# ZINZINBIN/Disruption-Prediciton-based-on-Multimodal-Deep-Learning

Hardware: AMD Instinct MI355X
Metric: clips/sec (fwd+bwd) R2Plus1D T=21 128x128 (higher is better)
Workload: dtype f32 storage; products as 3 fp16 (forward) / bf16 (backward) MFMAs on hi+lo splits, f32 accumulate; 1 GPU; R2Plus1D layer_sizes=[1,2,2,1] alpha=0.01, per-GPU clips (8,3,21,128,128) fp32, forward+FocalLoss(gamma=2)+backward+clip_grad_norm(1.0)+AdamW(2e-4), BN in train mode; per_gpu_batch=8, global_batch=8, parallelism=dp1

## Files before the change

disruption-prediciton-based-on-multimodal-deep-learning_amd/csrc/conv_patch.hip:

```cpp
#include "common.h"
#include <cstdlib>

#include "patch_common.h"

template <bool F16, int NT = 256>
__device__ __forceinline__ void stage_image(__amdgpu_buffer_rsrc_t src, int Cpitch, int c0, int cvalid4,
                                            const int* sG, int npix, int C8, unsigned magic, char* img, int pitch,
                                            int lo_off, bool prologue, const float* sScale, const float* sShift,
                                            float pslope, int t, bool presplit = false) {
  const int total = npix * C8;
  for (int base = 0; base < total; base += NT * 4) {
    float4 va[4], vb[4];
    int pix[4], c8s[4];
#pragma unroll
    for (int u = 0; u < 4; ++u) {
      const int item = min(base + u * NT + t, total - 1);
      const int pixel = mdiv(item, magic);
      const int c8 = item - pixel * C8;
      const int gp = sG[pixel];
      const bool in = gp >= 0 && c8 * 2 < cvalid4;
      const unsigned off = in ? (presplit ? (unsigned)(gp * C8 + c8) * 32u : (unsigned)(gp * Cpitch + c0 + c8 * 8) * 4u) : MD_OOB;
      va[u] = buf_load4(src, off);
      vb[u] = buf_load4(src, (in && (presplit || c8 * 2 + 1 < cvalid4)) ? off + 16u : MD_OOB);
      pix[u] = base + u * NT + t < total ? (pixel | (in ? 0 : 0x20000000)) : -1;
// ... 245 lines not shown
    if (fuse) {
      const int c = n0 + (j0 + j) * 16 + li;
      const bool cok = c < g.Cpd;
      const float csc = cok ? bw.scale[c] : 0.f, csh = cok ? bw.shift[c] : 0.f, cmu = cok ? bw.mean[c] : 0.f, cis = cok ? bw.invstd[c] : 0.f;
      float yv[2][4];
#pragma unroll
      for (int a = 0; a < 2; ++a)
#pragma unroll
        for (int r = 0; r < 4; ++r)
          yv[a][r] = __builtin_bit_cast(float, __builtin_amdgcn_raw_buffer_load_b32(yrs, colok ? goff[a][r] : MD_OOB, j * 64, 0));
#pragma unroll
      for (int a = 0; a < 2; ++a)
#pragma unroll
        for (int r = 0; r < 4; ++r) {
          const float pre = fmaf(yv[a][r], csc, csh);
          const float v = (acc[a][j][r] + prev[a][r]) * md_dleaky(pre, bw.slope);
          const float vm = v * gw[a][r];
          s1 += vm; s2 = fmaf(vm, (yv[a][r] - cmu) * cis, s2);
          __builtin_amdgcn_raw_buffer_store_b32(__builtin_bit_cast(unsigned, v), drs, colok ? goff[a][r] : MD_OOB, j * 64, 0);
        }
    } else {
#pragma unroll
      for (int a = 0; a < 2; ++a)
#pragma unroll
        for (int r = 0; r < 4; ++r) {
          const float v = acc[a][j][r];
          const float vm = v * gw[a][r];
          s1 += vm; s2 = fmaf(vm, v, s2);
          __builtin_amdgcn_raw_buffer_store_b32(__builtin_bit_cast(unsigned, v + prev[a][r]), drs, colok ? goff[a][r] : MD_OOB, j * 64, 0);
        }
    }
    if (stat_partial != nullptr) {
      s1 += __shfl_xor(s1, 16); s2 += __shfl_xor(s2, 16);
      s1 += __shfl_xor(s1, 32); s2 += __shfl_xor(s2, 32);
      if (lg == 0 && !dup) {
        red[(wr * 2 + 0) * (PNREP * 16) + (j0 + j) * 16 + li] = s1;
        red[(wr * 2 + 1) * (PNREP * 16) + (j0 + j) * 16 + li] = s2;
      }
    }
  }
  if (stat_partial != nullptr) {
    __syncthreads();
    if (t < ncols && n0 + t < g.Cpd) {
      float s1 = 0.f, s2 = 0.f;
#pragma unroll
      for (int w = 0; w < RG; ++w) {
        s1 += red[(w * 2 + 0) * (PNREP * 16) + t];
        s2 += red[(w * 2 + 1) * (PNREP * 16) + t];
      }
      float* sp = stat_partial + (size_t)blockIdx.x * 2 * g.Cpd;
      sp[n0 + t] = s1;
      sp[g.Cpd + n0 + t] = s2;
    }
  }
}

__device__ __forceinline__ float pack2_weight(const float* __restrict__ w, int n, int tap, int ch, int Cout, int Cin, int kwp,
                                              int kw_real, int shift, int taps_real) {
  const int sx = tap % kwp, row = tap / kwp;
  const int j = ch >> 2, c = ch & 3;
  const int dx = 2 * sx + j + shift;
  if (n < Cout && c < Cin && dx >= 0 && dx < kw_real) return w[((size_t)n * Cin + c) * taps_real + row * kw_real + dx];
  return 0.f;
}


struct ClassSpec { int c[3], tap0[3], kc[3], e[3]; };

static bool patch_build(const MdConvDesc* d, int dgrad, PGeom* out, size_t* lds_bytes, const ClassSpec* cls = nullptr,
                        int pers_wgs = 0, int pm_rows = PM, int npb_force = 0) {
  PGeom g;
  const bool sdg = !cls && dgrad && (d->st != 1 || d->sh != 1 || d->sw != 1);
  g.strided = sdg ? 1 : 0;
  if (sdg && (ilog2_exact(d->st) < 0 || ilog2_exact(d->sh) < 0 || ilog2_exact(d->sw) < 0)) return false;
  g.st = dgrad ? 1 : d->st; g.sh = dgrad ? 1 : d->sh; g.sw = dgrad ? 1 : d->sw;
  g.dst_ = d->st; g.dsh_ = d->sh; g.dsw_ = d->sw;
  g.lt = sdg ? ilog2_exact(d->st) : 0; g.lh = sdg ? ilog2_exact(d->sh) : 0; g.lw = sdg ? ilog2_exact(d->sw) : 0;
  g.oddmask = (g.lt ? ((1 << g.lt) - 1) : 0) | ((g.lh ? ((1 << g.lh) - 1) : 0) << 8) | ((g.lw ? ((1 << g.lw) - 1) : 0) << 16);
  g.kt = d->kt; g.padt = d->pt; g.padh = d->ph; g.padw = d->pw;
  const int cs = dgrad ? d->Cout : d->Cin, cd = dgrad ? d->Cin : d->Cout;
  g.Ts = dgrad ? d->To : d->Ti; g.Hs = dgrad ? d->Ho : d->Hi; g.Ws = dgrad ? d->Wo : d->Wi; g.Cps = md_cpad(cs);
  g.Td = dgrad ? d->Ti : d->To; g.Hd = dgrad ? d->Hi : d->Ho; g.Wd = dgrad ? d->Wi : d->Wo; g.Cpd = md_cpad(cd);
  g.kh = d->kh; g.kw = d->kw; g.khw = d->kh * d->kw; g.taps = d->kt * g.khw;
  if (!dgrad) { g.org_t = -d->pt; g.org_h = -d->ph; g.org_w = -d->pw; }
  else { g.org_t = d->pt - (d->kt - 1); g.org_h = d->ph - (d->kh - 1); g.org_w = d->pw - (d->kw - 1); }
  g.Tdf = g.Td; g.Hdf = g.Hd; g.Wdf = g.Wd; g.dmt = g.dmh = g.dmw = 1; g.dpt = g.dph = g.dpw = 0;
  int kt_eff = d->kt, kh_eff = d->kh;
  if (cls) {
    const int sd[3] = {d->st, d->sh, d->sw};
    int cd_[3];
    const int full[3] = {g.Td, g.Hd, g.Wd};
    for (int i = 0; i < 3; ++i) cd_[i] = full[i] > cls->c[i] ? (full[i] - cls->c[i] + sd[i] - 1) / sd[i] : 0;
    if (cd_[0] < 1 || cd_[1] < 1 || cd_[2] < 1) return false;
    g.Td = cd_[0]; g.Hd = cd_[1]; g.Wd = cd_[2];
    g.dmt = sd[0]; g.dmh = sd[1]; g.dmw = sd[2]; g.dpt = cls->c[0]; g.dph = cls->c[1]; g.dpw = cls->c[2];
    g.kt = cls->kc[0]; g.kh = cls->kc[1]; g.kw = cls->kc[2]; g.khw = g.kh * g.kw; g.taps = g.kt * g.khw;
    g.org_t = cls->e[0] - (cls->kc[0] - 1); g.org_h = cls->e[1] - (cls->kc[1] - 1); g.org_w = cls->e[2] - (cls->kc[2] - 1);
    kt_eff = g.kt; kh_eff = g.kh;
  }
  g.pack2 = 0; g.pk_shift = 0; g.pk_kw = d->kw;
  static const int no_pack2 = getenv("MD_PACK2") && atoi(getenv("MD_PACK2")) == 0;
  int kw_eff = cls ? g.kw : d->kw, sw_eff = g.sw;
  if (!dgrad && !no_pack2 && g.Cps == 4 && d->sw == 2 && (d->Wi & 1) == 0 && d->kw >= 2) {
    const int lo = -((d->pw + 1) / 2);
    const int num = d->kw - 1 - d->pw;
    const int hi = num >= 0 ? num / 2 : -((-num + 1) / 2);
// ... 318 lines not shown
int patch_pack(const MdConvDesc* d, int dgrad, const PatchPlan* p, const float* w, float* out, hipStream_t s) {
  (void)p;
  unsigned char handled = 0;
  const int rc = patch_pack_batch(1, &d, &dgrad, &w, &out, &handled, s);
  return rc ? rc : (handled ? MD_OK : MD_ERR_UNSUPPORTED);
}

static bool pers_can_fuse(const PersVariant& pv);
static PersBwd no_bwd() { PersBwd n; n.yraw = nullptr; n.scale = n.shift = n.mean = n.invstd = nullptr; n.slope = 1.f; return n; }
static int patch_launch_half(const PatchPlan* p, const float* src, const float* ps, const float* psh, float slope, const float* wp,
                             float* dst, float* stat, int accumulate, hipStream_t s, const PersBwd* bw) {
  const PGeom& g = p->gh;
  const PersBwd bwv = bw ? *bw : no_bwd();
  if ((accumulate >> 16) & 1) { if (!p->dgrad || g.pack2) return MD_ERR_UNSUPPORTED; }
  const int boxes = p->N * g.nbt * g.nby * g.nbx;
  int npb = p->half_npb;
  {
    static const int fill = getenv("MD_PATCH_FILL") ? atoi(getenv("MD_PATCH_FILL")) : 128;
    while (npb > 32 && boxes * md_cdiv(g.N16, npb) < 2 * fill) npb = md_round_up(md_cdiv(npb, 2), 16) < 32 ? 32 : md_round_up(md_cdiv(npb, 2), 16);
  }
  dim3 grid(boxes, md_cdiv(g.N16, npb));
  static const int dbg = getenv("MD_DBG") ? atoi(getenv("MD_DBG")) : 0;
  accumulate = (accumulate & 0x10001) | ((dbg & 0xff) << 8);
  const int nrep = npb / 16;
  const size_t lds = p->ldsh;
#define LAUNCH_HALF(F16_, NR_)                                                                                          \
  do {                                                                                                                  \
    static bool set_ = false;                                                                                           \
    if (!set_) {                                                                                                        \
      if (hipFuncSetAttribute((const void*)k_conv_patch<F16_, false, NR_, false, true>,                                 \
                              hipFuncAttributeMaxDynamicSharedMemorySize, 160 * 1024) != hipSuccess)                    \
        return MD_ERR_LAUNCH;                                                                                           \
      set_ = true;                                                                                                      \
    }                                                                                                                   \
    MD_KLAUNCH((k_conv_patch<F16_, false, NR_, false, true>), grid, dim3(256), lds, s, g, src, ps, psh, slope,          \
               (const uint4*)wp, dst, stat, accumulate, npb, bwv);                                                      \
  } while (0)
#define LAUNCH_HALF_NR(F16_)                                                                                            \
  switch (nrep) {                                                                                                       \
    case 2: LAUNCH_HALF(F16_, 2); break;                                                                                \
    case 3: LAUNCH_HALF(F16_, 3); break;                                                                                \
    case 4: LAUNCH_HALF(F16_, 4); break;                                                                                \
    case 5: LAUNCH_HALF(F16_, 5); break;                                                                                \
    case 6: LAUNCH_HALF(F16_, 6); break;                                                                                \
    case 7: LAUNCH_HALF(F16_, 7); break;                                                                                \
    case 8: LAUNCH_HALF(F16_, 8); break;                                                                                \
    default: LAUNCH_HALF(F16_, 9); break;                                                                               \
  }
  if (!p->dgrad) { LAUNCH_HALF_NR(true); } else { LAUNCH_HALF_NR(false); }
  MD_CHECK_LAUNCH();
  return MD_OK;
}

static int patch_launch_one(const PatchPlan* p, const PGeom& g, size_t lds, const PersVariant& pv, const float* src, const float* ps,
                            const float* psh, float slope, const float* wp, float* dst, float* stat, int accumulate,
                            const PersBwd* bw, hipStream_t s) {
  if ((accumulate >> 16) & 1) { if (!p->dgrad || g.pack2) return MD_ERR_UNSUPPORTED; }
  if (pv.on && (!bw || pers_can_fuse(pv))) {
    PersBwd none; none.yraw = nullptr; none.scale = none.shift = none.mean = none.invstd = nullptr; none.slope = 1.f;
    return pers_launch(pv.pg, pv.lds, pv.grid, !p->dgrad, src, ps, psh, slope, wp, dst, stat, accumulate, bw ? *bw : none, s);
  }
  if (pv.on && bw && pv.nsl > 0) {
    for (int k = 0; k < pv.nsl; ++k) {
      const int rc = pers_launch(pv.sl[k], pv.sl_lds[k], pv.grid, false, src, ps, psh, slope, wp, dst, stat, accumulate, *bw, s);
      if (rc != MD_OK) return rc;
    }
    return MD_OK;
  }
  if (bw && !p->dgrad) return MD_ERR_UNSUPPORTED;
  if (p->half && &g == &p->g) return patch_launch_half(p, src, ps, psh, slope, wp, dst, stat, accumulate, s, bw);
  const PersBwd bwv = bw ? *bw : no_bwd();
  int nchunks = md_cdiv(g.N16, PNREP * 16);
  const int boxes = p->N * g.nbt * g.nby * g.nbx;
  {
    static const int fill = getenv("MD_PATCH_FILL") ? atoi(getenv("MD_PATCH_FILL")) : 128;
    int wantc = md_cdiv(fill, boxes);
    if (wantc > g.N16 / 16) wantc = g.N16 / 16;
    if (wantc > nchunks) nchunks = wantc;
  }
  const int npb = md_round_up(md_cdiv(g.N16, nchunks), 16);
  dim3 grid(boxes, md_cdiv(g.N16, npb));
  {
    static const int padkb = getenv("MD_LDS_PAD_KB") ? atoi(getenv("MD_LDS_PAD_KB")) : 0;
    if (padkb && lds + (size_t)padkb * 1024 <= 160 * 1024) lds += (size_t)padkb * 1024; else if (padkb) lds = 160 * 1024;
  }
  static const int dbg = getenv("MD_DBG") ? atoi(getenv("MD_DBG")) : 0;
  accumulate = (accumulate & 0x10001) | ((dbg & 0xff) << 8);
  const int nrep = npb / 16;
  static const int w8_env = getenv("MD_PATCH_W8") ? atoi(getenv("MD_PATCH_W8")) : 1;
  const bool w8 = w8_env && !g.strided && nrep >= 2 && (lds > 80 * 1024 || w8_env == 2);
#define LAUNCH_PATCH(F16_, STR_, NR_, W8_)                                                                              \
  do {                                                                                                                  \
    static bool set_ = false;                                                                                           \
    if (!set_) {                                                                                                        \
      if (hipFuncSetAttribute((const void*)k_conv_patch<F16_, STR_, NR_, W8_>,                                          \
                              hipFuncAttributeMaxDynamicSharedMemorySize, 160 * 1024) != hipSuccess)                    \
        return MD_ERR_LAUNCH;                                                                                           \
      set_ = true;                                                                                                      \
    }                                                                                                                   \
    MD_KLAUNCH((k_conv_patch<F16_, STR_, NR_, W8_>), grid, dim3(W8_ ? 512 : 256), lds, s, g, src, ps, psh, slope,       \
               (const uint4*)wp, dst, stat, accumulate, npb, bwv);                                                      \
  } while (0)
#define LAUNCH_PATCH_NR(F16_, STR_, W8_)                                                                                \
  switch (nrep) {                                                                                                       \
    case 1: LAUNCH_PATCH(F16_, STR_, 1, false); break;                                                                  \
    case 2: LAUNCH_PATCH(F16_, STR_, 2, W8_); break;                                                                    \
    case 3: LAUNCH_PATCH(F16_, STR_, 3, W8_); break;                                                                    \
    case 4: LAUNCH_PATCH(F16_, STR_, 4, W8_); break;                                                                    \
    case 5: LAUNCH_PATCH(F16_, STR_, 5, W8_); break;                                                                    \
    case 6: LAUNCH_PATCH(F16_, STR_, 6, W8_); break;                                                                    \
    case 7: LAUNCH_PATCH(F16_, STR_, 7, W8_); break;                                                                    \
    case 8: LAUNCH_PATCH(F16_, STR_, 8, W8_); break;                                                                    \
    default: LAUNCH_PATCH(F16_, STR_, 9, W8_); break;                                                                   \
  }
  if (!p->dgrad) { if (w8) { LAUNCH_PATCH_NR(true, false, true); } else { LAUNCH_PATCH_NR(true, false, false); } }
  else if (!g.strided) { if (w8) { LAUNCH_PATCH_NR(false, false, true); } else { LAUNCH_PATCH_NR(false, false, false); } }
  else { LAUNCH_PATCH_NR(false, true, false); }
  MD_CHECK_LAUNCH();
  return MD_OK;
}

static bool pers_can_fuse(const PersVariant& pv) {
  static const int maxn = getenv("MD_FUSE_MAXN16") ? atoi(getenv("MD_FUSE_MAXN16")) : 48;
  return pv.on && pv.pg.g.N16 <= maxn && !(pv.pg.g.N16 == 48 && pv.pg.nit > 4) && !(pv.pg.g.N16 > 48 && pv.pg.nit > 4);
}
static bool fuse_per_box(const PersVariant& pv) {
  static const int patch_off = getenv("MD_FUSE_PATCH") && atoi(getenv("MD_FUSE_PATCH")) == 0;
  static const int pers_fallback_on = getenv("MD_FUSE_PERS_FALLBACK") && atoi(getenv("MD_FUSE_PERS_FALLBACK")) == 1;
  if (patch_off) return false;
  if (!pv.on) return true;
  return !pers_can_fuse(pv) && pers_fallback_on;
}
bool patch_can_fuse(const PatchPlan* p) {
  if (!p->dgrad) return false;
  auto ok = [](const PersVariant& pv) { return pers_can_fuse(pv) || (pv.on && pv.nsl > 0) || fuse_per_box(pv); };
  if (!p->ncls) return ok(p->pers);
  for (int c = 0; c < p->ncls; ++c) if (!ok(p->cls[c].pers)) return false;
  return true;
}
int patch_fused_blocks(const PatchPlan* p) {
  auto nb = [&](const PGeom& g, const PersVariant& pv) {
    if (pers_can_fuse(pv) || (pv.on && pv.nsl > 0)) return pers_blocks(pv.pg, pv.grid);
    if (p->half && &g == &p->g) return p->N * p->gh.nbt * p->gh.nby * p->gh.nbx;
// ... 150 lines not shown
```

disruption-prediciton-based-on-multimodal-deep-learning_amd/csrc/conv_pers.hip:

```cpp
#include "patch_common.h"
#include <cstdlib>
#include <cstdio>
#include <type_traits>

__device__ __forceinline__ void buf_store4(__amdgpu_buffer_rsrc_t r, unsigned off, f32x4 v) {
  __builtin_amdgcn_raw_buffer_store_b128(__builtin_bit_cast(__attribute__((__vector_size__(4 * sizeof(unsigned)))) unsigned, v), r, off, 0, 0);
}
__device__ __forceinline__ f32x4 buf_load4v(__amdgpu_buffer_rsrc_t r, unsigned off) {
  return __builtin_bit_cast(f32x4, __builtin_amdgcn_raw_buffer_load_b128(r, off, 0, 0));
}
__device__ __forceinline__ f32x4 buf_load4_pinned(__amdgpu_buffer_rsrc_t r, unsigned off) {
  return __builtin_bit_cast(f32x4, __builtin_amdgcn_raw_buffer_load_b128(r, off, 0, 0));
}

template <bool F16, bool FUSE, int NREP, int MAXI>
__global__ __launch_bounds__(512) void k_conv_pers(
    PersGeom pg, const float* __restrict__ src, const float* __restrict__ pscale, const float* __restrict__ pshift,
    float pslope, const uint4* __restrict__ wp, float* __restrict__ dst, float* __restrict__ stat_partial,
    int accumulate, PersBwd bw) {
  extern __shared__ __attribute__((aligned(16))) char sm[];
  const PGeom& g = pg.g;
  constexpr int NT = 512, TT = 256;
  const int t = threadIdx.x;
  const int wave = __builtin_amdgcn_readfirstlane(t >> 6);
// ... 299 lines not shown
    }
  }
#else
  {
    int* ctr = (int*)(sm + pg.off_sync) + team * 16;
    int target = 0;
    auto team_sync = [&]() {
      target += 4;
      __builtin_amdgcn_fence(__ATOMIC_RELEASE, "workgroup");
      if (lane == 0) __hip_atomic_fetch_add(ctr, 1, __ATOMIC_RELAXED, __HIP_MEMORY_SCOPE_WORKGROUP);
      while (__hip_atomic_load(ctr, __ATOMIC_RELAXED, __HIP_MEMORY_SCOPE_WORKGROUP) < target) __builtin_amdgcn_s_sleep(2);
      __builtin_amdgcn_fence(__ATOMIC_ACQUIRE, "workgroup");
    };
    while (cur < pg.nboxes) {
      do_matrix();
      team_sync();
      do_move();
      team_sync();
      cur += stride;
    }
    __syncthreads();
  }
#endif

  if (stats) {
    float* red = (float*)(sm + pg.off_red);
#pragma unroll
    for (int j = 0; j < NREP; ++j)
#pragma unroll
      for (int r = 0; r < 4; ++r) {
        float a1 = s1[j][r], a2 = s2[j][r];
#pragma unroll
        for (int m = 1; m < 16; m <<= 1) { a1 += __shfl_xor(a1, m); a2 += __shfl_xor(a2, m); }
        if (li == 0) {
          red[(wave * 2 + 0) * (PNREP * 16) + c0 + j * 16 + r] = a1;
          red[(wave * 2 + 1) * (PNREP * 16) + c0 + j * 16 + r] = a2;
        }
      }
    __syncthreads();
    if (t < g.N16 && pg.n0 + t < g.Cpd) {
      float a1 = 0.f, a2 = 0.f;
#pragma unroll
      for (int w = 0; w < 8; ++w) {
        a1 += red[(w * 2 + 0) * (PNREP * 16) + t];
        a2 += red[(w * 2 + 1) * (PNREP * 16) + t];
      }
      float* sp = stat_partial + (size_t)blockIdx.x * 2 * g.Cpd + pg.n0;
      sp[t] = a1;
      sp[g.Cpd + t] = a2;
    }
  }
}

static int pers_num_cus() {
  static int n = 0;
  if (!n) {
    int dev = 0; hipDeviceProp_t p;
    if (hipGetDevice(&dev) == hipSuccess && hipGetDeviceProperties(&p, dev) == hipSuccess && p.multiProcessorCount > 0) n = p.multiProcessorCount;
    else { (void)hipGetLastError(); n = 256; }
  }
  return n;
}

bool pers_finish(PersGeom* pg, size_t* lds_bytes, int* grid) {
  PGeom& g = pg->g;
  pg->nsteps = md_cdiv(g.Kc8, 4);
  { int u = pg->nsteps * 4; while ((u & 3) != 2) ++u; pg->bpitch = u * 16; }
  pg->nboxes = 0;
  pg->n0 = 0; pg->N16w = g.N16;
  pg->patch_bytes = (g.P * g.ppitch + 15) & ~15;
  size_t off = (size_t)2 * pg->patch_bytes;
  pg->off_red = 0;
  if (off < (size_t)8 * 2 * PNREP * 16 * 4) off = (size_t)8 * 2 * PNREP * 16 * 4;
  pg->off_bres = (int)off; off += (size_t)2 * g.N16 * pg->bpitch;
  pg->off_k = (int)off; off += (size_t)(pg->nsteps * 4 + 4) * 4;
  off = (off + 15) & ~(size_t)15;
  pg->off_row = (int)off; off += (size_t)PM * 8;
  pg->sc_stride = g.C8 * 8; pg->bn_stride = g.N16;
  pg->off_sc = (int)off; off += (size_t)2 * pg->sc_stride * 4;
  pg->off_bn = (int)off; off += (size_t)4 * pg->bn_stride * 4;
  off = (off + 15) & ~(size_t)15;
  pg->off_sync = (int)off; off += 128;
  if (off > (size_t)(160 * 1024)) return false;
  *lds_bytes = off;
  *grid = pers_num_cus();
  return true;
}

size_t pers_bres_bytes(int Kc8, int N16) {
  int u = md_cdiv(Kc8, 4) * 4; while ((u & 3) != 2) ++u;
  return (size_t)2 * N16 * u * 16;
}
size_t pers_fixed_bytes(int Cps, int N16) { return (size_t)PM * 8 + (size_t)(2 * (Cps + 8) + 4 * N16) * 4 + 256 + 144; }

int pers_launch(const PersGeom& pg, size_t lds, int grid, bool f16, const float* src, const float* ps, const float* psh, float slope,
                const float* wp, float* dst, float* stat, int accumulate, const PersBwd& bw, hipStream_t s) {
  const PGeom& g = pg.g;
  const int nrep = g.N16 / 16;
  const int nblk = pers_blocks(pg, grid);
  static const int dbg = getenv("MD_DBG") ? atoi(getenv("MD_DBG")) : 0;
  static const int xcd = getenv("MD_PERS_XCD") ? atoi(getenv("MD_PERS_XCD")) : 0;
  static const int early = getenv("MD_PERS_EARLY") ? atoi(getenv("MD_PERS_EARLY")) : 0;
  accumulate = (accumulate & 0x10001) | ((dbg & 0xff) << 8) | (xcd ? 0x40000 : 0) | (early ? 0x80000 : 0);
#define LAUNCH_PERS(F16_, FUSE_, NR_, MX_)                                                                              \
  do {                                                                                                                  \
    static bool set_ = false;                                                                                           \
    if (!set_) {                                                                                                        \
// ... 31 lines not shown
```

disruption-prediciton-based-on-multimodal-deep-learning_amd/csrc/patch_common.h:

```cpp
#pragma once
#include "common.h"

typedef __bf16 bf16x8 __attribute__((ext_vector_type(8)));
typedef __bf16 bf16x2 __attribute__((ext_vector_type(2)));
typedef float f32x2 __attribute__((ext_vector_type(2)));

#define PM 128
#define PNREP 9
#define PB_PITCH 160
#define PMAXC 320

struct PGeom {
  int Ts, Hs, Ws, Cps;
  int Td, Hd, Wd, Cpd;
  int kh, kw, khw, taps;
  int org_t, org_h, org_w;
  int st, sh, sw;
  int strided;
  int dst_, dsh_, dsw_;
  int lt, lh, lw, oddmask;
  int kt, padt, padh, padw;
  int zero_off;
  int bt, by, bx, byx;
  int nbt, nby, nbx;
// ... 62 lines not shown
  } else {
#pragma unroll
    for (int i = 0; i < 4; ++i) {
      const f32x2 x = {v[2 * i], v[2 * i + 1]};
      const f32x2 pre = __builtin_elementwise_fma(x, s[i], h[i]);
      const f32x2 t = pre * sl;
      v[2 * i] = pre[0] > 0.f ? pre[0] : t[0]; v[2 * i + 1] = pre[1] > 0.f ? pre[1] : t[1];
    }
  }
}
__device__ __forceinline__ void zero8(float* v) {
#pragma unroll
  for (int e = 0; e < 8; ++e) v[e] = 0.f;
}

__device__ __forceinline__ int mdiv(int x, unsigned magic) { return magic ? (int)__umulhi((unsigned)x, magic) : x; }

#define MD_OOB 0x80000000u
__device__ __forceinline__ __amdgpu_buffer_rsrc_t make_rsrc(const void* p, unsigned bytes) {
  return __builtin_amdgcn_make_buffer_rsrc(const_cast<void*>(p), 0, bytes, 0x00020000);
}
__device__ __forceinline__ float4 buf_load4(__amdgpu_buffer_rsrc_t r, unsigned off) {
  const f32x4 f = __builtin_bit_cast(f32x4, __builtin_amdgcn_raw_buffer_load_b128(r, off, 0, 0));
  return make_float4(f[0], f[1], f[2], f[3]);
}

template <bool F16>
__device__ __forceinline__ f32x4 mma(uint4 a, uint4 b, f32x4 c) {
  if (F16) return __builtin_amdgcn_mfma_f32_16x16x32_f16(__builtin_bit_cast(f16x8, a), __builtin_bit_cast(f16x8, b), c, 0, 0, 0);
  return __builtin_amdgcn_mfma_f32_16x16x32_bf16(__builtin_bit_cast(bf16x8, a), __builtin_bit_cast(bf16x8, b), c, 0, 0, 0);
}


#define PERS_MAXI 8
struct PersGeom {
  PGeom g;
  int nboxes;
  int nsteps;
  int bpitch;
  int off_bres;
  int off_k, off_row, off_sc, off_red, off_bn, off_sync;
  int nit;
  int patch_bytes;
  int sc_stride, bn_stride;
  unsigned m_nbx, m_nby, m_nbt;
  int n0, N16w;
};
struct PersBwd {
  const float* yraw;
  const float* scale; const float* shift; const float* mean; const float* invstd;
  float slope;
};
bool pers_finish(PersGeom* pg, size_t* lds_bytes, int* grid);
static inline int pers_blocks(const PersGeom& pg, int grid) { const int need = (pg.nboxes + 1) / 2; return grid < need ? grid : need; }
size_t pers_bres_bytes(int Kc8, int N16);
size_t pers_fixed_bytes(int Cps, int N16);
int pers_launch(const PersGeom& pg, size_t lds, int grid, bool f16, const float* src, const float* ps, const float* psh, float slope,
                const float* wp, float* dst, float* stat, int accumulate, const PersBwd& bw, hipStream_t s);

#include <cstdlib>
static int pitch_for(int C8) {
  int u = C8;
  while ((u & 3) != 2) ++u;
  static const int add = getenv("MD_PITCH_ADD") ? atoi(getenv("MD_PITCH_ADD")) : 0;
  return (u + add) * 16;
}

static bool choose_box(int T, int H, int W, int kt, int kh, int kw, int st, int sh, int sw, int dgrad, int maxP, int softP,
                       int* bt, int* by, int* bx, int pm = PM) {
  double best = 1e300;
  bool found = false;
  auto pdim = [&](int b, int k, int s) { return dgrad ? (b + k - 2) / s + 2 : (b - 1) * s + k; };
  for (int t = 1; t <= T && t <= 32; ++t) {
    for (int x = 1; x <= pm; x *= 2) {
      const int xe = x >= W ? W : x;
      int ymax = pm / (t * xe);
      if (ymax >= 1) {
        if (ymax > H) ymax = H;
        for (int y = ymax; y >= 1; y = (y > 4 ? y / 2 : y - 1)) {
          const double boxes = (double)md_cdiv(T, t) * md_cdiv(H, y) * md_cdiv(W, xe);
          const long long patch = (long long)pdim(t, kt, st) * pdim(y, kh, sh) * pdim(xe, kw, sw);
          if (patch > maxP) continue;
          double cost = boxes * (pm + 0.6 * (double)patch);
          if (patch > softP) cost *= 1.25;
          if (cost < best) { best = cost; *bt = t; *by = y; *bx = xe; found = true; }
        }
      }
      if (x >= W) break;
    }
  }
  return found;
}

static unsigned magic_of(int d) { return d <= 1 ? 0u : (unsigned)(0x100000000ull / (unsigned)d) + 1u; }
static int ilog2_exact(int v) { int l = 0; while ((1 << l) < v) ++l; return (1 << l) == v ? l : -1; }
```

disruption-prediciton-based-on-multimodal-deep-learning_amd/src/_native.py:

```python
from __future__ import annotations

import ctypes as C
import os
import threading

import torch

_HERE = os.path.dirname(os.path.abspath(__file__))
LIB_PATH = os.path.join(os.path.dirname(_HERE), "csrc", "libmi355x_disrupt.so")

c_float_p = C.POINTER(C.c_float)
c_void_p = C.c_void_p


class MdConvDesc(C.Structure):
    _fields_ = [(n, C.c_int32) for n in
                ("N", "Ti", "Hi", "Wi", "Cin", "To", "Ho", "Wo", "Cout", "kt", "kh", "kw", "st", "sh", "sw", "pt", "ph", "pw")]


class MdActView(C.Structure):
    _fields_ = [("data", c_void_p), ("scale", c_void_p), ("shift", c_void_p), ("slope", C.c_float)]


class MdTrainStepArgs(C.Structure):
    _fields_ = ([(n, C.c_int32) for n in ("B", "Hd", "K", "loss_kind")] +
                [(n, c_void_p) for n in ("x", "target", "w", "gamma", "beta", "rmean", "rvar", "dw", "dgamma", "dbeta",
                                         "w0", "b0", "hgamma", "hbeta", "w1", "b1", "hrmean", "hrvar",
                                         "dw0", "db0", "dhgamma", "dhbeta", "dw1", "db1")] +
                [(n, C.c_float) for n in ("head_alpha", "head_eps", "head_momentum", "gamma_or_s")] +
                [(n, c_void_p) for n in ("class_weight", "margins", "feat", "dfeat", "logits", "dlogits", "head_save", "loss", "pred",
                                         "workspace", "counters")] +
                [("ncounters", C.c_int32), ("opt_nchunks", C.c_int32)] +
                [(n, c_void_p) for n in ("opt_tensors", "opt_chunks", "opt_partial")] +
                [(n, C.c_float) for n in ("max_norm", "lr", "beta1", "beta2", "eps", "weight_decay")] +
                [("opt_step", C.c_int64), ("ok_flag", c_void_p)])


_P = c_void_p
_I32, _I64, _F, _SZ = C.c_int32, C.c_int64, C.c_float, C.c_size_t
_DESC, _VIEW = C.POINTER(MdConvDesc), C.POINTER(MdActView)
SIGNATURES = {
    "md_version": (C.c_int, [C.POINTER(C.c_char_p)]),
    "md_set_exact_fp32": (C.c_int, [C.c_int]),
    "md_get_exact_fp32": (C.c_int, []),
    "md_set_pers_grid": (C.c_int, [C.c_int]),
    "md_set_wgrad_form": (C.c_int, [C.c_int]),
    "md_conv_wpack_fwd_floats": (_SZ, [_DESC]),
    "md_conv_wpack_dgrad_floats": (_SZ, [_DESC]),
    "md_conv_pack_weights": (C.c_int, [_DESC, _P, _P, _P, _P]),
    "md_conv_pack_weights_batch": (C.c_int, [_I32, _P, _P, _P, _P, _P]),
    "md_conv_fwd_stat_blocks": (_I32, [_DESC]),
    "md_conv_fwd": (C.c_int, [_DESC, _VIEW, _P, _P, _P, _P]),
    "md_conv_dgrad": (C.c_int, [_DESC, _P, _P, _P, C.c_int, _P]),
    "md_conv_wgrad_workspace_floats": (_SZ, [_DESC]),
    "md_conv_wgrad": (C.c_int, [_DESC, _VIEW, _P, _P, _P, _P]),
    "md_bn_finalize": (C.c_int, [_P, _I32, _I32, _I64, _P, _P, _F, _F, _P, _P, _P, _P, _P, _P, _P]),
    "md_bn_eval_params": (C.c_int, [_I32, _P, _P, _P, _P, _F, _P, _P, _P, _P, _P]),
    "md_bn_act": (C.c_int, [_VIEW, _I64, _I32, _P, _P]),
    "md_residual_fwd": (C.c_int, [_VIEW, _VIEW, _F, _I64, _I32, _P, _P]),
    "md_bn_bwd_blocks": (_I32, [_I64, _I32]),
    "md_bn_bwd_reduce": (C.c_int, [_P, _VIEW, _VIEW, _F, _P, _P, _I64, _I32, _P, _P]),
    "md_bn_bwd_finalize": (C.c_int, [_P, _I32, _I32, _I64, _P, _P, _P, _P]),
    "md_bn_bwd_apply": (C.c_int, [_P, _VIEW, _VIEW, _F, _P, _P, _P, _I64, _I32, _P, _P, _P]),
    "md_conv_dgrad_bnred_blocks": (_I32, [_DESC]),
    "md_conv_dgrad_bnred": (C.c_int, [_DESC, _P, _P, _P, C.c_int, _VIEW, _P, _P, _P, _P]),
    "md_bn_bwd_apply_g": (C.c_int, [_P, _VIEW, _P, _P, _P, _I64, _I32, _P, _P]),
    "md_conv_split_dy_ok": (C.c_int, [_DESC, C.c_int]),
    "md_bn_bwd_apply_fmt": (C.c_int, [_P, C.c_int, _VIEW, _VIEW, _F, _P, _P, _P, _I64, _I32, _P, C.c_int, _P, _P]),
    "md_bn_bwd_apply_fused": (C.c_int, [_P, C.c_int, _VIEW, _VIEW, _F, _P, _P, _P, _I32, _I64, _P, _P, _I64, _I32, _P, _P, _P]),
    "md_conv_dgrad_fmt": (C.c_int, [_DESC, _P, C.c_int, _P, _P, C.c_int, _VIEW, _P, _P, _P, _P]),
    "md_conv_wgrad_fmt": (C.c_int, [_DESC, _VIEW, _P, C.c_int, _P, _P, _P]),
    "md_conv_wgrad_fmt2": (C.c_int, [_DESC, _VIEW, C.c_int, _P, C.c_int, _P, _P, _P]),
    "md_conv_wgrad_xsplit_ok": (C.c_int, [_DESC]),
    "md_bn_act_split_floats": (_SZ, [_I64, _I32]),
    "md_bn_act_split": (C.c_int, [_VIEW, _I64, _I32, _P, _P]),
    "md_nchw_to_cl": (C.c_int, [_P, _I32, _I32, _I64, _P, _P]),
    "md_cl_to_nchw": (C.c_int, [_P, _I32, _I32, _I64, _P, _P]),
    "md_cat_cl": (C.c_int, [_P, _I32, _P, _I32, _I64, _P, _P]),
    "md_split_cl": (C.c_int, [_P, _I32, _I32, _I64, _P, _P, _P]),
    "md_avgpool_fwd": (C.c_int, [_P, _I32, _I32, _I64, _P, _P]),
    "md_avgpool_bwd": (C.c_int, [_P, _I32, _I32, _I64, _P, _P]),
    "md_head_save_floats": (_SZ, [_I32, _I32, _I32]),
    "md_head_fwd": (C.c_int, [_P, _I32, _I32, _I32, _I32, _P, _P, _P, _P, _P, _P, _F, _F, _F, C.c_int, _P, _P, _P, _P, _P]),
    "md_head_bwd": (C.c_int, [_P, _P, _I32, _I32, _I32, _I32, _P, _P, _P, _F, _P, _P, _P, _P, _P, _P, _P, _P, _P]),
    "md_softmax_loss": (C.c_int, [_I32, _P, _P, _I32, _I32, _P, _P, _F, _P, _P, _P, _P]),
    "md_plan_create": (C.c_int, [_I32, _I32, _I32, _I32, C.POINTER(_I32), _F, C.POINTER(_P)]),
    "md_plan_destroy": (None, [_P]),
    "md_plan_num_units": (_I32, [_P]),
    "md_plan_unit_desc": (C.c_int, [_P, _I32, _DESC]),
    "md_plan_workspace_bytes": (_SZ, [_P]),
    "md_plan_unit_layout": (C.c_int, [_P, _I32, C.POINTER(_SZ), C.POINTER(_SZ), C.POINTER(_I64), C.POINTER(_I32)]),
    "md_plan_num_z": (_I32, [_P]),
    "md_plan_z_layout": (C.c_int, [_P, _I32, C.POINTER(_SZ), C.POINTER(_I64), C.POINTER(_I32)]),
    "md_plan_forward": (C.c_int, [_P, _P, _P, _P, _P, _P, _P, C.c_int, _P, _P, _P]),
    "md_plan_backward": (C.c_int, [_P, _P, _P, _P, _P, _P, _P, _P, _P]),
    "md_plan_backward_range": (C.c_int, [_P, _P, _P, _P, _P, _P, _P, _P, _I32, _I32, _P]),
    "md_plan_feat_dim": (_I32, [_P]),
    "md_plan_train_step": (C.c_int, [_P, C.POINTER(MdTrainStepArgs), _P]),
# ... 107 lines not shown
```

include/mi355x_disrupt.h:

```cpp
#ifndef MI355X_DISRUPT_H
#define MI355X_DISRUPT_H

#include <stddef.h>
#include <stdint.h>

#ifdef __cplusplus
extern "C" {
#endif

#define MD_OK 0
#define MD_ERR_BAD_SHAPE (-1)
#define MD_ERR_UNSUPPORTED (-2)
#define MD_ERR_WORKSPACE (-3)
#define MD_ERR_LAUNCH (-4)
#define MD_ERR_NULL (-5)

int md_version(const char** arch_out);

int md_set_exact_fp32(int on);
int md_get_exact_fp32(void);
int md_set_pers_grid(int n);
int md_set_wgrad_form(int first_form_only);

typedef struct MdConvDesc {
  int32_t N, Ti, Hi, Wi, Cin;
  int32_t To, Ho, Wo, Cout;
  int32_t kt, kh, kw;
  int32_t st, sh, sw;
  int32_t pt, ph, pw;
} MdConvDesc;

typedef struct MdActView {
  const float* data;
  const float* scale;
  const float* shift;
  float slope;
} MdActView;

static inline int32_t md_cpad(int32_t c) { return (c + 3) & ~3; }

size_t md_conv_wpack_fwd_floats(const MdConvDesc* d);
size_t md_conv_wpack_dgrad_floats(const MdConvDesc* d);
int md_conv_pack_weights(const MdConvDesc* d, const float* w, float* wpack_fwd, float* wpack_dgrad, void* stream);
int md_conv_pack_weights_batch(int32_t n, const MdConvDesc* descs, const float* const* w, float* const* wpack_fwd,
                               float* const* wpack_dgrad, void* stream);

int32_t md_conv_fwd_stat_blocks(const MdConvDesc* d);

int md_conv_fwd(const MdConvDesc* d, const MdActView* x, const float* wpack_fwd, float* y_raw,
                float* stat_partial, void* stream);

int md_conv_dgrad(const MdConvDesc* d, const float* dy_raw, const float* wpack_dgrad, float* dx,
                  int accumulate, void* stream);

size_t md_conv_wgrad_workspace_floats(const MdConvDesc* d);
int md_conv_wgrad(const MdConvDesc* d, const MdActView* x, const float* dy_raw, float* dw, float* workspace,
                  void* stream);

int md_bn_finalize(const float* stat_partial, int32_t blocks, int32_t C, int64_t count,
                   const float* gamma, const float* beta, float eps, float momentum,
                   float* running_mean, float* running_var,
                   float* mean, float* invstd, float* scale, float* shift, void* stream);

int md_bn_eval_params(int32_t C, const float* gamma, const float* beta, const float* running_mean,
                      const float* running_var, float eps, float* mean, float* invstd, float* scale,
                      float* shift, void* stream);

int md_bn_act(const MdActView* x, int64_t rows, int32_t C, float* out, void* stream);

int md_residual_fwd(const MdActView* skip, const MdActView* main, float alpha, int64_t rows, int32_t C,
                    float* z, void* stream);

int32_t md_bn_bwd_blocks(int64_t rows, int32_t C);
int md_bn_bwd_reduce(const float* dA, const MdActView* main, const MdActView* skip, float alpha,
// ... 228 lines not shown
```

Measured before the change: 1415 clips/s.

## Add persistent patch-conv kernel that prefetches next tile's patch and weights

Adds a persistent variant of the patch convolution kernel. A grid sized to CU count times residency loops over (box, column-chunk) work items. While it computes the current item, it issues global loads for the next item's input patch and weight slice into registers, then commits them to LDS after the epilogue, so loads overlap MFMA work across items. It is enabled by default for non-strided, non-class cases with W8 or nrep==2, and falls back to the old kernel when unsupported. This adds register pressure from the prefetch buffers and a reduced grid, which may lower occupancy. Epilogue stats are written per box.

```diff
diff --git a/disruption-prediciton-based-on-multimodal-deep-learning_amd/csrc/conv_patch.hip b/disruption-prediciton-based-on-multimodal-deep-learning_amd/csrc/conv_patch.hip
--- a/disruption-prediciton-based-on-multimodal-deep-learning_amd/csrc/conv_patch.hip
+++ b/disruption-prediciton-based-on-multimodal-deep-learning_amd/csrc/conv_patch.hip
@@ -321,6 +321,314 @@
       sp[n0 + t] = s1;
       sp[g.Cpd + n0 + t] = s2;
     }
+  }
+}
+
+template <bool F16, int NREP, bool W8, int NI>
+__global__ __launch_bounds__(W8 ? 512 : 256) void k_conv_patch_pers(
+    PGeom g, const float* __restrict__ src, const float* __restrict__ pscale, const float* __restrict__ pshift,
+    float pslope, const uint4* __restrict__ wp, float* __restrict__ dst, float* __restrict__ stat_partial,
+    int accumulate, int n_per_blk, PersBwd bw, int nboxes, int off_red) {
+  extern __shared__ __attribute__((aligned(16))) char sm[];
+  char* sP = sm;
+  char* sB = sm + g.off_b;
+  int* sK = (int*)(sm + g.off_koffs);
+  int4* sR = (int4*)(sm + g.off_rows);
+  float* sScale = (float*)(sm + g.off_scale);
+  float* sShift = sScale + PMAXC;
+  float* red = (float*)(sm + off_red);
+
+  const int t = threadIdx.x;
+  constexpr int NT = W8 ? 512 : 256;
+  constexpr int RG = 4;
+  constexpr int NW = W8 ? (NREP + 1) / 2 : NREP;
+  const int lane = t & 63, wave = t >> 6;
+  const int wr = wave & (RG - 1), wc = wave / RG;
+  const int j0 = wc ? NREP - NW : 0;
+  const int li = lane & 15, lg = lane >> 4;
+  const bool prologue = pscale != nullptr;
+  const bool presplit = (accumulate >> 16) & 1;
+  accumulate &= 1;
+  const int nitems = nboxes * ((g.N16 + n_per_blk - 1) / n_per_blk);
+
+  struct Item { int box, n, t0, y0, x0, n0, ncols; };
+  auto decode = [&](int item) {
+    Item it;
+    it.box = item % nboxes;
+    it.n0 = (item / nboxes) * n_per_blk;
+    it.ncols = min(n_per_blk, g.N16 - it.n0);
+    int b = it.box;
+    const int xb = b % g.nbx; b /= g.nbx;
+    const int yb = b % g.nby; b /= g.nby;
+    const int tb = b % g.nbt; it.n = b / g.nbt;
+    it.t0 = tb * g.bt; it.y0 = yb * g.by; it.x0 = xb * g.bx;
+    return it;
+  };
+  auto build_rows = [&](const Item& it) {
+    if (t < 32 * RG) {
+      const int rt = mdiv(t, g.m_byx); const int r = t - rt * g.byx;
+      const int ry = mdiv(r, g.m_bx); const int rx = r - ry * g.bx;
+      const bool v = (rt < g.bt) && (it.t0 + rt < g.Td) && (it.y0 + ry < g.Hd) && (it.x0 + rx < g.Wd);
+      int4 ri;
+      ri.x = v ? ((rt * g.st * g.py + ry * g.sh) * g.px + rx * g.sw) * g.ppitch : 0;
+      ri.y = v ? ((it.n * g.Tdf + (it.t0 + rt) * g.dmt + g.dpt) * g.Hdf + (it.y0 + ry) * g.dmh + g.dph) * g.Wdf + (it.x0 + rx) * g.dmw + g.dpw
+               : -1;
+      ri.z = 0; ri.w = 0;
+      sR[t] = ri;
+    }
+  };
+
+  const int total = g.P * g.C8;
+  const __amdgpu_buffer_rsrc_t srs =
+      make_rsrc(src, presplit ? (unsigned)(g.src_bytes / (g.Cps * 4u)) * (unsigned)g.C8 * 32u : g.src_bytes);
+  const int cvalid4 = presplit ? 2 * g.C8 : g.Cps >> 2;
+  float4 pa[NI], pb[NI];
+  int pinf[NI];
+  auto issue_patch = [&](const Item& it, bool live) {
+#pragma unroll
+    for (int u = 0; u < NI; ++u) {
+      if (u * NT >= total) break;
+      const int q = u * NT + t;
+      const int item = min(q, total - 1);
+      const int pixel = mdiv(item, g.magicC8);
+      const int c8 = item - pixel * g.C8;
+      const int ppt = mdiv(pixel, g.m_pyx); const int r = pixel - ppt * g.pyx;
+      const int ppy = mdiv(r, g.m_px); const int ppx = r - ppy * g.px;
+      const int st = it.t0 * g.st + g.org_t + ppt, sy = it.y0 * g.sh + g.org_h + ppy, sx = it.x0 * g.sw + g.org_w + ppx;
+      const bool v = ((unsigned)st < (unsigned)g.Ts) && ((unsigned)sy < (unsigned)g.Hs) && ((unsigned)sx < (unsigned)g.Ws);
+      const int gp = ((it.n * g.Ts + st) * g.Hs + sy) * g.Ws + sx;
+      const bool in = v && c8 * 2 < cvalid4;
+      const bool req = live && in && q < total;
+      const unsigned off = req ? (presplit ? (unsigned)(gp * g.C8 + c8) * 32u : (unsigned)(gp * g.Cps + c8 * 8) * 4u) : MD_OOB;
+      pa[u] = buf_load4(srs, off);
+      pb[u] = buf_load4(srs, (req && (presplit || c8 * 2 + 1 < cvalid4)) ? off + 16u : MD_OOB);
+      pinf[u] = q < total ? (pixel | (c8 << 16) | (in ? 0 : 0x20000000)) : -1;
+    }
+  };
+  auto commit_patch = [&]() {
+#pragma unroll
+    for (int u = 0; u < NI; ++u) {
+      if (u * NT >= total || pinf[u] == -1) continue;
+      const int pixel = pinf[u] & 0xffff, c8 = (pinf[u] >> 16) & 0xff;
+      float v[8] = {pa[u].x, pa[u].y, pa[u].z, pa[u].w, pb[u].x, pb[u].y, pb[u].z, pb[u].w};
+      if (prologue) {
+        const float* sc = sScale + c8 * 8; const float* sh = sShift + c8 * 8;
+        const f32x4 sc0 = *(const f32x4*)sc, sc1 = *(const f32x4*)(sc + 4), sh0 = *(const f32x4*)sh, sh1 = *(const f32x4*)(sh + 4);
+        bn_leaky8(v, sc0, sc1, sh0, sh1, pslope);
+        if (pinf[u] & 0x20000000) zero8(v);
+      }
+      uint4 hi, lo;
+      if (presplit) { hi = __builtin_bit_cast(uint4, pa[u]); lo = __builtin_bit_cast(uint4, pb[u]); }
+      else if (F16) split8_f16(v, hi, lo); else split8(v, hi, lo);
+      char* d = sP + pixel * g.ppitch + c8 * 16;
+      *(uint4*)d = hi;
+      *(uint4*)(d + g.lo_off) = lo;
+    }
+  };
+
+  constexpr int NB = (NREP * 128 + NT - 1) / NT;
+  uint4 rb[2][NB];
+  const int blo = n_per_blk * PB_PITCH;
+  auto load_b = [&](int kb, int n0, int ncols) {
+#pragma unroll
+    for (int h = 0; h < 2; ++h) {
+      const uint4* base = wp + ((size_t)(kb * 2 + h) * g.N16 + n0) * 8;
+#pragma unroll
+      for (int i = 0; i < NB; ++i) {
+        const uint4 v = base[min(t + NT * i, ncols * 8 - 1)];
+        rb[h][i] = v;
+      }
+    }
+  };
+  auto store_b = [&]() {
+#pragma unroll
+    for (int h = 0; h < 2; ++h)
+#pragma unroll
+      for (int i = 0; i < NB; ++i) {
+        const int c = t + NT * i;
+        const uint4 v = rb[h][i];
+        if (c < n_per_blk * 8) *(uint4*)(sB + h * blo + (c >> 3) * PB_PITCH + (c & 7) * 16) = v;
+      }
+  };
+
+  int item = blockIdx.x;
+  if (item >= nitems) return;
+  Item cur = decode(item);
+
+  for (int q = t; q < g.nstages * 8; q += NT) {
+    int ko = 0;
+    if (q < g.Kc8) {
+      const int tap = mdiv(q, g.magicC8); const int c8 = q - tap * g.C8;
+      const int dt = mdiv(tap, g.m_khw); const int r = tap - dt * g.khw;
+      const int dy = mdiv(r, g.m_kw); const int dx = r - dy * g.kw;
+      ko = ((dt * g.py + dy) * g.px + dx) * g.ppitch + c8 * 16;
+    }
+    sK[q] = ko;
+  }
+  if (prologue) for (int c = t; c < g.C8 * 8; c += NT) {
+    const int cs = g.pack2 ? (c & 3) : c;
+    sScale[c] = c < g.Cps ? pscale[cs] : 0.f; sShift[c] = c < g.Cps ? pshift[cs] : 0.f;
+  }
+  build_rows(cur);
+  issue_patch(cur, true);
+  load_b(0, cur.n0, cur.ncols);
+  __syncthreads();
+  commit_patch();
+  store_b();
+
+  const char* bbase = sB + (j0 * 16 + li) * PB_PITCH + lg * 16;
+  const int nsteps = g.nstages * 2;
+  const bool fuse = !F16 && bw.yraw != nullptr;
+  const __amdgpu_buffer_rsrc_t drs = make_rsrc(dst, g.dst_bytes);
+  const __amdgpu_buffer_rsrc_t yrs = make_rsrc(fuse ? bw.yraw : dst, g.dst_bytes);
+  for (;;) {
+    const int next = item + (int)gridDim.x;
+    const bool more = next < nitems;
+    const Item nxt = decode(more ? next : item);
+    __syncthreads();
+
+    const int rp0 = sR[wr * 32 + li].x, rp1 = sR[wr * 32 + 16 + li].x;
+    f32x4 acc[2][NW];
+#pragma unroll
+    for (int a = 0; a < 2; ++a)
+#pragma unroll
+      for (int j = 0; j < NW; ++j) acc[a][j] = (f32x4){0.f, 0.f, 0.f, 0.f};
+    uint4 fa[2][4];
+    auto load_a = [&](int ko, uint4* f) {
+      f[0] = *(const uint4*)(sP + rp0 + ko); f[1] = *(const uint4*)(sP + g.lo_off + rp0 + ko);
+      f[2] = *(const uint4*)(sP + rp1 + ko); f[3] = *(const uint4*)(sP + g.lo_off + rp1 + ko);
+    };
+    load_a(sK[lg], fa[0]);
+    int ko_next = sK[4 + lg];
+    auto stage = [&](int kb, bool first) __attribute__((always_inline)) {
+      if (!first) {
+        __syncthreads();
+        store_b();
+        __syncthreads();
+      }
+      const bool last = kb + 1 == g.nstages;
+      load_b(last ? 0 : kb + 1, last ? nxt.n0 : cur.n0, last ? nxt.ncols : cur.ncols);
+      if (first) issue_patch(nxt, more);
+      uint4 fb[2][2];
+      fb[0][0] = *(const uint4*)bbase; fb[0][1] = *(const uint4*)(bbase + blo);
+      __builtin_amdgcn_sched_group_barrier(0x100, 2, 0);
+#pragma unroll
+      for (int s = 0; s < 2; ++s) {
+        load_a(ko_next, fa[s ^ 1]);
+        ko_next = sK[min(kb * 2 + s + 2, nsteps - 1) * 4 + lg];
+        const uint4 ah0 = fa[s][0], al0 = fa[s][1], ah1 = fa[s][2], al1 = fa[s][3];
+#pragma unroll
+        for (int j = 0; j < NW; ++j) {
+          const int cb = (s * NW + j) & 1;
+          const bool mj = j + 1 < NW || s == 0;
+          if (mj) {
+            const int jn = j + 1 < NW ? j + 1 : 0, sn = j + 1 < NW ? s : 1;
+            const char* bp = bbase + jn * 16 * PB_PITCH + sn * 64;
+            fb[cb ^ 1][0] = *(const uint4*)bp; fb[cb ^ 1][1] = *(const uint4*)(bp + blo);
+          }
+          const uint4 bh = fb[cb][0], bl = fb[cb][1];
+          acc[0][j] = mma<F16>(al0, bh, acc[0][j]);
+          acc[1][j] = mma<F16>(al1, bh, acc[1][j]);
+          acc[0][j] = mma<F16>(ah0, bl, acc[0][j]);
+          acc[1][j] = mma<F16>(ah1, bl, acc[1][j]);
+          acc[0][j] = mma<F16>(ah0, bh, acc[0][j]);
+          acc[1][j] = mma<F16>(ah1, bh, acc[1][j]);
+          if (j == 0 && mj) __builtin_amdgcn_sched_group_barrier(0x100, 7, 0);
+          else if (j == 0) __builtin_amdgcn_sched_group_barrier(0x100, 5, 0);
+          else if (mj) __builtin_amdgcn_sched_group_barrier(0x100, 2, 0);
+          __builtin_amdgcn_sched_group_barrier(0x008, 6, 0);
+        }
+      }
+    };
+    stage(0, true);
+    if (g.nstages > 1) stage(1, false);
+    for (int kb = 2; kb < g.nstages; ++kb) stage(kb, false);
+
+    unsigned goff[2][4];
+    float gw[2][4];
+#pragma unroll
+    for (int a = 0; a < 2; ++a)
+#pragma unroll
+      for (int r = 0; r < 4; ++r) {
+        const int gi = sR[wr * 32 + a * 16 + lg * 4 + r].y;
+        goff[a][r] = gi >= 0 ? (unsigned)(gi * g.Cpd + cur.n0 + j0 * 16 + li) * 4u : MD_OOB;
+        gw[a][r] = gi >= 0 ? 1.f : 0.f;
+      }
+    __syncthreads();
+    if (more) {
+      commit_patch();
+      store_b();
+      build_rows(nxt);
+    }
+#pragma unroll
+    for (int j = 0; j < NW; ++j) {
+      const bool dup = W8 && (NREP & 1) && wc == 1 && j == 0;
+      const bool colok = !dup && cur.n0 + (j0 + j) * 16 + li < g.Cpd;
+      float s1 = 0.f, s2 = 0.f;
+      float prev[2][4] = {{0.f, 0.f, 0.f, 0.f}, {0.f, 0.f, 0.f, 0.f}};
+      if (accumulate) {
+#pragma unroll
+        for (int a = 0; a < 2; ++a)
+#pragma unroll
+          for (int r = 0; r < 4; ++r)
+            prev[a][r] = __builtin_bit_cast(float, __builtin_amdgcn_raw_buffer_load_b32(drs, colok ? goff[a][r] : MD_OOB, j * 64, 0));
+      }
+      if (fuse) {
+        const int c = cur.n0 + (j0 + j) * 16 + li;
+        const bool cok = c < g.Cpd;
+        const float csc = cok ? bw.scale[c] : 0.f, csh = cok ? bw.shift[c] : 0.f, cmu = cok ? bw.mean[c] : 0.f, cis = cok ? bw.invstd[c] : 0.f;
+        float yv[2][4];
+#pragma unroll
+        for (int a = 0; a < 2; ++a)
+#pragma unroll
+          for (int r = 0; r < 4; ++r)
+            yv[a][r] = __builtin_bit_cast(float, __builtin_amdgcn_raw_buffer_load_b32(yrs, colok ? goff[a][r] : MD_OOB, j * 64, 0));
+#pragma unroll
+        for (int a = 0; a < 2; ++a)
+#pragma unroll
+          for (int r = 0; r < 4; ++r) {
+            const float pre = fmaf(yv[a][r], csc, csh);
+            const float v = (acc[a][j][r] + prev[a][r]) * md_dleaky(pre, bw.slope);
+            const float vm = v * gw[a][r];
+            s1 += vm; s2 = fmaf(vm, (yv[a][r] - cmu) * cis, s2);
+            __builtin_amdgcn_raw_buffer_store_b32(__builtin_bit_cast(unsigned, v), drs, colok ? goff[a][r] : MD_OOB, j * 64, 0);
+          }
+      } else {
+#pragma unroll
+        for (int a = 0; a < 2; ++a)
+#pragma unroll
+          for (int r = 0; r < 4; ++r) {
+            const float v = acc[a][j][r];
+            const float vm = v * gw[a][r];
+            s1 += vm; s2 = fmaf(vm, v, s2);
+            __builtin_amdgcn_raw_buffer_store_b32(__builtin_bit_cast(unsigned, v + prev[a][r]), drs, colok ? goff[a][r] : MD_OOB, j * 64, 0);
+          }
+      }
+      if (stat_partial != nullptr) {
+        s1 += __shfl_xor(s1, 16); s2 += __shfl_xor(s2, 16);
+        s1 += __shfl_xor(s1, 32); s2 += __shfl_xor(s2, 32);
+        if (lg == 0 && !dup) {
+          red[(wr * 2 + 0) * (PNREP * 16) + (j0 + j) * 16 + li] = s1;
+          red[(wr * 2 + 1) * (PNREP * 16) + (j0 + j) * 16 + li] = s2;
+        }
+      }
+    }
+    if (stat_partial != nullptr) {
+      __syncthreads();
+      if (t < cur.ncols && cur.n0 + t < g.Cpd) {
+        float s1 = 0.f, s2 = 0.f;
+#pragma unroll
+        for (int w = 0; w < RG; ++w) {
+          s1 += red[(w * 2 + 0) * (PNREP * 16) + t];
+          s2 += red[(w * 2 + 1) * (PNREP * 16) + t];
+        }
+        float* sp = stat_partial + (size_t)cur.box * 2 * g.Cpd;
+        sp[cur.n0 + t] = s1;
+        sp[g.Cpd + cur.n0 + t] = s2;
+      }
+    }
+    if (!more) break;
+    item = next; cur = nxt;
   }
 }
 
@@ -745,6 +1053,71 @@
   return MD_OK;
 }
 
+static int patch_persist_env() { const char* e = getenv("MD_PATCH_PERSIST"); return e ? (atoi(e) != 0 ? 1 : 0) : 1; }
+static std::atomic<int> g_patch_persist{patch_persist_env()};
+static std::atomic<int> g_patch_persist_grid{0};
+extern "C" int md_set_patch_persist(int on) { return g_patch_persist.exchange(on ? 1 : 0); }
+extern "C" int md_set_patch_persist_grid(int n) { return g_patch_persist_grid.exchange(n > 0 ? n : 0); }
+
+static constexpr int patch_pers_ni(int nrep) { return nrep >= 7 ? 5 : 8; }
+#define PATCH_PERS_RED (4 * 2 * PNREP * 16 * 4)
+
+static int patch_pers_residency(const void* k, int nt, size_t lds) {
+  static std::mutex mu;
+  static std::map<std::pair<const void*, size_t>, int> cache;
+  std::lock_guard<std::mutex> lock(mu);
+  auto it = cache.find({k, lds});
+  if (it != cache.end()) return it->second;
+  int nb = 0;
+  if (hipFuncSetAttribute(k, hipFuncAttributeMaxDynamicSharedMemorySize, 160 * 1024) != hipSuccess ||
+      hipOccupancyMaxActiveBlocksPerMultiprocessor(&nb, k, nt, lds) != hipSuccess || nb < 1) {
+    (void)hipGetLastError();
+    nb = 1;
+  }
+  cache[{k, lds}] = nb;
+  return nb;
+}
+
+template <bool F16, int NR, bool W8>
+static int launch_patch_pers(const PGeom& g, size_t lds, int boxes, int npb, const float* src, const float* ps, const float* psh,
+                             float slope, const float* wp, float* dst, float* stat, int accumulate, const PersBwd& bw, hipStream_t s) {
+  constexpr int NT = W8 ? 512 : 256;
+  const auto k = k_conv_patch_pers<F16, NR, W8, patch_pers_ni(NR)>;
+  const size_t off_red = (lds + 15) & ~(size_t)15;
+  const size_t lds_p = off_red + PATCH_PERS_RED;
+  if (lds_p > (size_t)160 * 1024) return MD_ERR_UNSUPPORTED;
+  const int wgs = patch_pers_residency((const void*)k, NT, lds_p);
+  const int per_box = (size_t)160 * 1024 / lds >= 2 ? 2 : 1;
+  if (wgs < per_box) return MD_ERR_UNSUPPORTED;
+  const int items = boxes * md_cdiv(g.N16, npb);
+  const int forced = g_patch_persist_grid.load();
+  int grid = forced ? forced : pers_num_cus() * wgs;
+  if (grid > items) grid = items;
+  MD_KLAUNCH(k, dim3(grid), dim3(NT), lds_p, s, g, src, ps, psh, slope, (const uint4*)wp, dst, stat, accumulate, npb, bw, boxes,
+             (int)off_red);
+  MD_CHECK_LAUNCH();
+  return MD_OK;
+}
+
+static int patch_launch_pers(const PGeom& g, size_t lds, bool w8, bool f16, int nrep, int boxes, int npb, const float* src,
+                             const float* ps, const float* psh, float slope, const float* wp, float* dst, float* stat, int accumulate,
+                             const PersBwd& bw, hipStream_t s) {
+  if (md_cdiv(g.P * g.C8, w8 ? 512 : 256) > patch_pers_ni(nrep)) return MD_ERR_UNSUPPORTED;
+#define PERS_ARGS g, lds, boxes, npb, src, ps, psh, slope, wp, dst, stat, accumulate, bw, s
+#define PERS_CASE(NR_) \
+  case NR_: return f16 ? launch_patch_pers<true, NR_, true>(PERS_ARGS) : launch_patch_pers<false, NR_, true>(PERS_ARGS)
+  if (!w8) {
+    if (nrep != 2) return MD_ERR_UNSUPPORTED;
+    return f16 ? launch_patch_pers<true, 2, false>(PERS_ARGS) : launch_patch_pers<false, 2, false>(PERS_ARGS);
+  }
+  switch (nrep) {
+    PERS_CASE(2); PERS_CASE(3); PERS_CASE(4); PERS_CASE(5); PERS_CASE(6); PERS_CASE(7); PERS_CASE(8); PERS_CASE(9);
+    default: return MD_ERR_UNSUPPORTED;
+  }
+#undef PERS_CASE
+#undef PERS_ARGS
+}
+
 static int patch_launch_one(const PatchPlan* p, const PGeom& g, size_t lds, const PersVariant& pv, const float* src, const float* ps,
                             const float* psh, float slope, const float* wp, float* dst, float* stat, int accumulate,
                             const PersBwd* bw, hipStream_t s) {
@@ -782,6 +1155,10 @@
   const int nrep = npb / 16;
   static const int w8_env = getenv("MD_PATCH_W8") ? atoi(getenv("MD_PATCH_W8")) : 1;
   const bool w8 = w8_env && !g.strided && nrep >= 2 && (lds > 80 * 1024 || w8_env == 2);
+  if (g_patch_persist.load() && !g.strided && !p->ncls && (w8 || nrep == 2)) {
+    const int rc = patch_launch_pers(g, lds, w8, !p->dgrad, nrep, boxes, npb, src, ps, psh, slope, wp, dst, stat, accumulate, bwv, s);
+    if (rc != MD_ERR_UNSUPPORTED) return rc;
+  }
 #define LAUNCH_PATCH(F16_, STR_, NR_, W8_)                                                                              \
   do {                                                                                                                  \
     static bool set_ = false;                                                                                           \
diff --git a/disruption-prediciton-based-on-multimodal-deep-learning_amd/csrc/conv_pers.hip b/disruption-prediciton-based-on-multimodal-deep-learning_amd/csrc/conv_pers.hip
--- a/disruption-prediciton-based-on-multimodal-deep-learning_amd/csrc/conv_pers.hip
+++ b/disruption-prediciton-based-on-multimodal-deep-learning_amd/csrc/conv_pers.hip
@@ -375,7 +375,7 @@
   }
 }
 
-static int pers_num_cus() {
+int pers_num_cus() {
   static int n = 0;
   if (!n) {
     int dev = 0; hipDeviceProp_t p;
diff --git a/disruption-prediciton-based-on-multimodal-deep-learning_amd/csrc/patch_common.h b/disruption-prediciton-based-on-multimodal-deep-learning_amd/csrc/patch_common.h
--- a/disruption-prediciton-based-on-multimodal-deep-learning_amd/csrc/patch_common.h
+++ b/disruption-prediciton-based-on-multimodal-deep-learning_amd/csrc/patch_common.h
@@ -138,6 +138,7 @@
   float slope;
 };
 bool pers_finish(PersGeom* pg, size_t* lds_bytes, int* grid);
+int pers_num_cus();
 static inline int pers_blocks(const PersGeom& pg, int grid) { const int need = (pg.nboxes + 1) / 2; return grid < need ? grid : need; }
 size_t pers_bres_bytes(int Kc8, int N16);
 size_t pers_fixed_bytes(int Cps, int N16);
diff --git a/disruption-prediciton-based-on-multimodal-deep-learning_amd/src/_native.py b/disruption-prediciton-based-on-multimodal-deep-learning_amd/src/_native.py
--- a/disruption-prediciton-based-on-multimodal-deep-learning_amd/src/_native.py
+++ b/disruption-prediciton-based-on-multimodal-deep-learning_amd/src/_native.py
@@ -44,6 +44,8 @@
     "md_set_exact_fp32": (C.c_int, [C.c_int]),
     "md_get_exact_fp32": (C.c_int, []),
     "md_set_pers_grid": (C.c_int, [C.c_int]),
+    "md_set_patch_persist": (C.c_int, [C.c_int]),
+    "md_set_patch_persist_grid": (C.c_int, [C.c_int]),
     "md_set_wgrad_form": (C.c_int, [C.c_int]),
     "md_conv_wpack_fwd_floats": (_SZ, [_DESC]),
     "md_conv_wpack_dgrad_floats": (_SZ, [_DESC]),
diff --git a/include/mi355x_disrupt.h b/include/mi355x_disrupt.h
--- a/include/mi355x_disrupt.h
+++ b/include/mi355x_disrupt.h
@@ -20,6 +20,8 @@
 int md_set_exact_fp32(int on);
 int md_get_exact_fp32(void);
 int md_set_pers_grid(int n);
+int md_set_patch_persist(int on);
+int md_set_patch_persist_grid(int n);
 int md_set_wgrad_form(int first_form_only);
 
 typedef struct MdConvDesc {
```

Result: slower. 1390 clips/s, median of 2 (-1.7%).
